# ahmetumutdurmus/zaremba

Hardware: NVIDIA H100
Metric: tokens/sec (and valid perplexity) Large-LSTM 1500h at 1/2/4/8 H100 vs ref CPU (higher is better)
Workload: dtype f16 operands, f32 accumulate/state

## Files before the change

zaremba_b200/csrc/engine_tc.cu:

```cuda
#include "engine.h"
#include <stdlib.h>
#include <string.h>

#include "tc_kernels.h"

struct GridBarrier {
    unsigned int* word = nullptr;
    unsigned int base = 0;
    template <typename Launch>
    int claim(int T, int nCTA, cudaStream_t s, Launch&& launch) {
        const unsigned int arrivals = (unsigned int)T * (unsigned int)nCTA;
        if (base > 0xF0000000u - arrivals) {
            ZRB_CUDA(cudaMemsetAsync(word, 0, sizeof(unsigned int), s));
            base = 0;
        }
        ZRB_TRY(launch(word, base));
        base += arrivals;
        return ZRB_OK;
    }
};

struct zrb_tc_state {
    int Xp[ZRB_MAX_LAYERS + 1] = {}, G4p[ZRB_MAX_LAYERS] = {}, Vp = 0;
    int Fp = 0;
// ... 213 lines not shown
    zrb_tc_state::WhhImage w;
    if (wd_mask(c, l).active) {
        w.kind = zrb_tc_state::kWhhMasked;
        w.seed = c->wd_seed; w.step = c->step; w.p = c->p_wd;
    }
    return w;
}
static bool whh_current(const zrb_ctx* c, int l) {
    const zrb_tc_state::WhhImage &have = c->tc->whh_img[l], want = whh_wanted(c, l);
    if (have.kind != want.kind) return false;
    return want.kind == zrb_tc_state::kWhhRaw || (have.seed == want.seed && have.step == want.step && have.p == want.p);
}

static int tc_pack_whh(zrb_ctx* c, const float* W, int l, bool row_image, cudaStream_t s) {
    const int H = c->width[l + 1];
    const MaskSrc m = wd_mask(c, l);
    const WeightImages w = c->tc->w_hh_images(l, whh_wanted(c, l), row_image);
    if (w.row) ZRB_TRY(convert_pad_f16(W, H, w.row, w.ld, 4 * H, H, 1.f, s, m));
    if (w.fwd) ZRB_TRY(pack_whh_fwd(W, w.fwd, H, *w.fplan, s, m));
    if (w.bwd) ZRB_TRY(pack_whh_bwd(W, w.bwd, H, *w.bplan, s, m));
    return ZRB_OK;
}

static size_t params_bytes(const zrb_ctx* c) { return c->experts ? sizeof(zrb_mos_params) : sizeof(zrb_params); }
static void note_packed(zrb_ctx* c, const zrb_params* p) {
    zrb_tc_state* t = c->tc;
    t->packed_version = c->weights_version;
    memcpy(&t->packed_params, p, params_bytes(c));
}

static int tc_pack_weights(zrb_ctx* c, const zrb_params* p, cudaStream_t s) {
    zrb_tc_state* t = c->tc;
    if (t->packed_version == c->weights_version && !memcmp(&t->packed_params, p, params_bytes(c))) return ZRB_OK;
    ProfScope ps(c, ZRB_PROF_PACK, s);
    const int L = c->cfg.layers, V = c->cfg.vocab;
    for (int l = 0; l < L; ++l) {
        const int In = c->width[l], H = c->width[l + 1];
        ZRB_TRY(convert_pad_f16(p->w_ih[l], In, t->w_ih_h[l], t->Xp[l], 4 * H, In, 1.f, s));
        ZRB_TRY(tc_pack_whh(c, p->w_hh[l], l, true, s));
    }
    const int F = c->experts ? c->width[0] : c->width[L];
    ZRB_TRY(convert_pad_f16(p->fc_w, F, t->fc_w_h, t->Fp, V, F, 1.f, s));
    if (c->experts) {
        const int K = c->experts, H = c->width[L];
        const zrb_mos_params* mp = mos_of(p);
        ZRB_TRY(convert_pad_f16(mp->latent_w, H, t->head_w_h, t->Xp[L], K * c->width[0], H, 1.f, s));
        ZRB_TRY(convert_pad_f16(mp->prior_w, H, t->head_w_h + (size_t)t->Ua * t->Xp[L], t->Xp[L], K, H, 1.f, s));
    }
    note_packed(c, p);
    return ZRB_OK;
}

struct WeightMatrix {
    int i, rows, cols, item;
    enum { kWih, kWhh, kFcW, kPrior, kLatent } kind;
};
struct WeightMatrices {
    WeightMatrix m[2 * ZRB_MAX_LAYERS + 3];
    int n = 0;
    const WeightMatrix* begin() const { return m; }
    const WeightMatrix* end() const { return m + n; }
    const WeightMatrix& fc_w() const { return m[n - 1]; }
};
static WeightMatrices tc_matrices(const zrb_ctx* c) {
    const int L = c->cfg.layers, V = c->cfg.vocab, K = c->experts;
    WeightMatrices ms;
    for (int l = 0; l < L; ++l) {
        const int In = c->width[l], H = c->width[l + 1];
        ms.m[ms.n++] = {1 + 4 * l, 4 * H, In, l, WeightMatrix::kWih};
        ms.m[ms.n++] = {2 + 4 * l, 4 * H, H, l, WeightMatrix::kWhh};
    }
    if (K) {
        ms.m[ms.n++] = {3 + 4 * L, K, c->width[L], L, WeightMatrix::kPrior};
        ms.m[ms.n++] = {4 + 4 * L, K * c->width[0], c->width[L], L, WeightMatrix::kLatent};
    }
    ms.m[ms.n++] = {1 + 4 * L, V, K ? c->width[0] : c->width[L], L, WeightMatrix::kFcW};
    return ms;
}
static WeightImages tc_images(zrb_ctx* c, const WeightMatrix& m, const zrb_tc_state::WhhImage& whh) {
    zrb_tc_state* t = c->tc;
    switch (m.kind) {
        case WeightMatrix::kWhh: return t->w_hh_images(m.item, whh);
        case WeightMatrix::kWih: return t->w_ih_images(m.item);
        case WeightMatrix::kFcW: return t->fc_w_images();
        case WeightMatrix::kPrior: return t->row_image(t->head_w_h + (size_t)t->Ua * t->Xp[m.item], t->Xp[m.item]);
        default: return t->row_image(t->head_w_h, t->Xp[m.item]);
    }
}
static TensorList tc_without_matrices(const zrb_ctx* c, const TensorList& tl) {
    TensorList rest = tl;
    for (const WeightMatrix& m : tc_matrices(c)) rest.n[m.i] = 0;
    return rest;
}
static void tc_images_current(zrb_ctx* c, const zrb_params* p) {
    zrb_tc_state* t = c->tc;
    t->wg_ok = false;
    c->weights_version++;
    note_packed(c, p);
}

static int tc_update_matrix(zrb_ctx* c, const WeightMatrix& m, const UpdateStep& st, int pdl_smem, cudaStream_t s) {
    zrb_tc_state::WhhImage whh;
    if (st.train() && c->p_wd > 0.f) whh.kind = zrb_tc_state::kWhhStale;
    const WeightImages img = tc_images(c, m, whh);
    float *p = st.tl.p[m.i], *g = st.tl.g[m.i];
    switch (st.kind) {
        case UpdateStep::kSgd:
            return update_pack(p, g, m.rows, m.cols, st.lr, c->scalars, img, c->keep_clipped, s, pdl_smem);
        case UpdateStep::kSgdAvg:
            return update_pack_avg(p, g, st.avg.a[m.i], st.avg.mu, st.avg.first, m.rows, m.cols, st.lr, c->scalars, img,
                                   c->keep_clipped, s, pdl_smem);
        case UpdateStep::kAdam:
            return update_pack_adam(p, g, st.adam.m[m.i], st.adam.v[m.i], st.adam.k, m.rows, m.cols, c->scalars, img,
                                    c->keep_clipped, s, pdl_smem);
        case UpdateStep::kDyn:
            return update_pack_dyn(p, g, st.tg[m.i], st.r[m.i], m.rows, m.cols, st.dyn, img, s);
        case UpdateStep::kSwap:
            return swap_pack(p, st.avg.a[m.i], m.rows, m.cols, img, s);
    }
    return ZRB_E_INVALID;
}

static int tc_issue_update(zrb_ctx* c, int item, int pdl_smem, cudaStream_t s) {
    zrb_tc_state* t = c->tc;
    if (!(t->upd_pending & (1u << item))) return ZRB_OK;
    t->upd_pending &= ~(1u << item);
    for (const WeightMatrix& m : tc_matrices(c))
        if (m.item == item) ZRB_TRY(tc_update_matrix(c, m, t->upd, pdl_smem, s));
    return ZRB_OK;
}

int tc_flush_updates(zrb_ctx* c, cudaStream_t s) {
    zrb_tc_state* t = c->tc;
    if (!t || !t->upd_pending) return ZRB_OK;
    ProfScope ps(c, ZRB_PROF_CLIP_SGD, s);
    for (int item = 1; item <= c->cfg.layers; ++item) ZRB_TRY(tc_issue_update(c, item, 0, s));
    return ZRB_OK;
}

static int tc_mos_head(zrb_ctx* c, const zrb_params* p, int rows, float* logp, cudaStream_t s) {
    zrb_tc_state* t = c->tc;
    const int L = c->cfg.layers, V = c->cfg.vocab, K = c->experts, E = c->width[0], H = c->width[L];
    const int N = c->T * c->B, Xl = t->Xp[L], Ep = pad64(E);
    ProfScope ps(c, ZRB_PROF_PROJ_FWD, s);
    Gemm head;
    head.A = {t->x_h[L] + (size_t)(N - rows) * Xl, Xl}; head.B = {t->head_w_h, Xl};
    head.C = t->ua; head.ldc = t->HW; head.M = rows; head.N = t->Ua + K; head.K = H;
    ZRB_TRY(gemm_f16_tc(head, s));
    ZRB_TRY(mos_latent_fwd(t->ua, t->HW, mos_of(p)->latent_b, t->lat_h, Ep, rows, K, E, N - rows, mos_mask(c), s));
    Gemm logits;
    logits.A = {t->lat_h, Ep}; logits.B = {t->fc_w_h, t->Fp};
    logits.C = t->logits; logits.ldc = V; logits.M = rows * K; logits.N = V; logits.K = E; logits.bias = p->fc_b;
    ZRB_TRY(gemm_f16_tc(logits, s));
    ZRB_TRY(mos_lse(t->logits, rows * K, V, t->lse, s));
    if (logp) ZRB_TRY(mos_logp(t->logits, t->lse, t->ua, t->HW, t->Ua, rows, K, V, logp, V, s));
    return ZRB_OK;
}

int tc_forward(zrb_ctx* c, const zrb_params* p, const int64_t* x, const zrb_states* in, const zrb_states* out,
               float* scores, cudaStream_t s, bool last_only) {
    zrb_tc_state* t = c->tc;
    const int L = c->cfg.layers, V = c->cfg.vocab, T = c->T, B = c->B, N = T * B;
    const bool ride = t->upd_pending && t->in_train_step && t->fplan[0].ok && pdl_beside_rec(c);
    if (t->upd_pending && !ride) ZRB_TRY(tc_flush_updates(c, s));
    ZRB_TRY(tc_pack_weights(c, p, s));
    {
        FwdPrep fp = {};
        for (int l = 0; l < L; ++l) {
            fp.in_h[l] = in->h[l]; fp.in_c[l] = in->c[l]; fp.h0s[l] = c->h0s[l]; fp.c0s[l] = c->c0s[l];
            fp.hprev_h[l] = t->hprev_h[l]; fp.h0_img[l] = t->fplan[l].ok ? t->h0_img[l] : nullptr;
            fp.rm[l] = rec_mask(c, l);
            fp.H[l] = c->width[l + 1]; fp.Hp[l] = t->Xp[l + 1]; fp.GB[l] = t->fplan[l].GBi; fp.Kc[l] = t->fplan[l].Kc;
        }
        fp.x = x; fp.x_saved = c->x_saved;
        fp.L = L; fp.B = B; fp.N = N;
        ZRB_TRY(fwd_prep(fp, s));
    }
    ZRB_TRY(zoneout_draw(c, s));
    {
        ProfScope ps(c, ZRB_PROF_EMBED_FWD, s);
        const bool through = ride && c->tied && (t->upd_pending & (1u << L));
        ZRB_TRY(embed_dropout_fwd(p->embed_w, x, nullptr, t->x_h[0], t->Xp[0], N, c->width[0], V, site_mask(c, 0), ed_mask(c), s,
                                  through ? t->upd.tl.g[tc_matrices(c).fc_w().i] : nullptr, t->upd.lr, c->scalars));
    }
    for (int l = 0; l < L; ++l) {
        const int In = c->width[l], H = c->width[l + 1], Xi = t->Xp[l], Hp = t->Xp[l + 1];
        const size_t bh = (size_t)B * H * sizeof(float);
        const RecPlan& fplan = t->fplan[l];
        float* G = c->gates[l];
        if (!whh_current(c, l)) {
            ProfScope ps(c, ZRB_PROF_PACK, s);
            ZRB_TRY(tc_pack_whh(c, p->w_hh[l], l, false, s));
        }
        {
            ProfScope ps(c, ZRB_PROF_GEMM_IN, s);
            Gemm xw;
            xw.A = {t->x_h[l], Xi}; xw.B = {t->w_ih_h[l], Xi};
            xw.C = G; xw.ldc = 4 * H; xw.M = N; xw.N = 4 * H; xw.K = In; xw.bias = p->b_ih[l]; xw.bias2 = p->b_hh[l];
            ZRB_TRY(gemm_f16_tc(xw, s));
        }
        MaskSrc m = site_mask(c, l + 1), rm = rec_mask(c, l);
        const ZoneoutSrc zo = zoneout_src(c, l);
        const bool reg_h = t->in_train_step && reg_on(c) && l == L - 1;
        ProfScope ps(c, ZRB_PROF_REC_FWD, s);
        if (fplan.ok) {
            ZRB_TRY(t->fwd_bar.claim(T, fplan.nCTA, s, [&](unsigned int* word, unsigned int base) {
                RecFwdArgs a = {};
                a.w_img = t->w_img_f[l]; a.h0_img = t->h0_img[l]; a.h_img = t->h_img; a.gates = G; a.c0 = c->c0s[l];
                a.cst = c->cst[l]; a.h_last = out->h[l]; a.c_last = out->c[l]; a.hprev_h = t->hprev_h[l];
                a.y_h = t->x_h[l + 1]; a.h_f32 = reg_h ? c->hraw[l] : nullptr; a.counter = word; a.base = base;
                a.T = T; a.B = B; a.H = H; a.Hp = Hp; a.m = m; a.rm = rm; a.trace = t->trace;
                a.zo = zo; a.h0 = c->h0s[l]; a.ctil = c->ctil[l];
                return lstm_rec_fwd(fplan, tc_watchdog(c), a, s);
            }));
            if (ride) ZRB_TRY(tc_issue_update(c, l + 1, fplan.beside_smem, s));
            continue;
        }
        for (int tt = 0; tt < T; ++tt) {
            const float* c_prev = tt ? c->cst[l] + (size_t)(tt - 1) * B * H : c->c0s[l];
            float* Gt = G + (size_t)tt * B * 4 * H;
            Gemm hw;
            hw.A = {t->hprev_h[l] + (size_t)tt * B * Hp, Hp}; hw.B = {t->w_hh_h[l], Hp};
            hw.C = Gt; hw.ldc = 4 * H; hw.M = B; hw.N = 4 * H; hw.K = H; hw.accumulate = true;
            ZRB_TRY(gemm_f16_tc(hw, s));
            const float* h_prev = tt ? c->hraw[l] + (size_t)(tt - 1) * B * H : c->h0s[l];
            ZRB_TRY(lstm_cell_fwd_tc(Gt, c_prev, c->cst[l] + (size_t)tt * B * H, c->hraw[l] + (size_t)tt * B * H,
                                     t->hprev_h[l] + (size_t)(tt + 1) * B * Hp, t->x_h[l + 1] + (size_t)tt * B * Hp, Hp, B,
                                     H, (int64_t)tt * B * H, (int64_t)N * H, m, rm, s, zo.on ? &zo : nullptr, h_prev,
                                     zo.on ? c->ctil[l] + (size_t)tt * B * H : nullptr));
        }
        ZRB_CUDA(cudaMemcpyAsync(out->h[l], c->hraw[l] + (size_t)(T - 1) * B * H, bh, cudaMemcpyDeviceToDevice, s));
        ZRB_CUDA(cudaMemcpyAsync(out->c[l], c->cst[l] + (size_t)(T - 1) * B * H, bh, cudaMemcpyDeviceToDevice, s));
    }
    if (scores && c->experts) return tc_mos_head(c, p, last_only ? B : N, t->head_loss_only ? nullptr : scores, s);
    if (scores) {
        ProfScope ps(c, ZRB_PROF_PROJ_FWD, s);
        const int rows = last_only ? B : N;
        const int Xl = t->Xp[L];
        Gemm proj;
        proj.A = {t->x_h[L] + (size_t)(N - rows) * Xl, Xl}; proj.B = {t->fc_w_h, Xl};
        proj.C = scores; proj.ldc = V; proj.M = rows; proj.N = V; proj.K = c->width[L]; proj.bias = p->fc_b;
        ZRB_TRY(gemm_f16_tc(proj, s));
    }
    return ZRB_OK;
}

const __half* tc_last_layer_image(const zrb_ctx* c) { return c->tc->x_h[c->cfg.layers]; }

static float* wgrad_slots(zrb_ctx* c, int n) {
    zrb_tc_state* t = c->tc;
    if (!t->wg_ok) return nullptr;
    if (t->wg_slots + n > kNormGemm) {
        t->wg_ok = false;
        return nullptr;
    }
    float* out = c->partials + norm_partials_base() + kNormExtra + t->wg_slots;
    t->wg_slots += n;
    return out;
}
static float* wgrad_sumsq(zrb_ctx* c, const Gemm& d) { return wgrad_slots(c, gemm_f16_tc_sumsq_slots(d).first); }

static int tc_mos_backward(zrb_ctx* c, const zrb_params* g, float* dY, cudaStream_t s) {
    zrb_tc_state* t = c->tc;
    const int L = c->cfg.layers, V = c->cfg.vocab, N = c->T * c->B, H = c->width[L], K = c->experts, E = c->width[0];
    const int NK = N * K, Xl = t->Xp[L], Vp = t->Vp, Ep = pad64(E);
// ... 365 lines not shown
    dw.dual.B = t->hprev_h[0]; dw.dual.C = dw_hh; dw.dual.N = H; dw.dual.ldb = Hp; dw.dual.ldc = H;
    ZRB_TRY(gemm_f16_tc(dw, s));
    c->layer_fwd_ok = false;
    return ZRB_OK;
}

int tc_rec_trace(zrb_ctx* c, long long* h_out, int max_entries) {
    if (!c->tc || !c->tc->trace) { set_error("set ZRB_REC_TRACE=1 before creating the context"); return ZRB_E_STATE; }
    int n = 2 * (8 + c->cfg.max_seq * 8);
    if (n > max_entries) n = max_entries;
    ZRB_CUDA(cudaDeviceSynchronize());
    ZRB_CUDA(cudaMemcpy(h_out, c->tc->trace, (size_t)n * sizeof(long long), cudaMemcpyDeviceToHost));
    return n;
}

int tc_apply_update(zrb_ctx* c, const zrb_params* p, const UpdateStep& st, float max_norm, float* norm_out,
                    cudaStream_t s) {
    zrb_tc_state* t = c->tc;
    const TensorList& tl = st.tl;
    const int E = c->width[0], V = c->cfg.vocab, L = c->cfg.layers;
    const bool adam = st.kind == UpdateStep::kAdam;
    ZRB_TRY(tc_flush_updates(c, s));
    ProfScope ps(c, st.kind == UpdateStep::kSwap ? ZRB_PROF_PACK : ZRB_PROF_CLIP_SGD, s);
    TensorList rest = tc_without_matrices(c, tl);
    bool lazy = false;
    if (st.train()) {
        const bool rows_only = !c->tied && c->emb_sparse && c->emb_prev_grad == tl.g[0] && c->emb_prev_n > 0;
        const bool gemm_norm = t->wg_ok && t->wg_key == tl.g[tc_matrices(c).fc_w().i];
        if (rows_only && !adam) rest.n[0] = 0;
        TensorList dense = gemm_norm ? rest : tl;
        if (rows_only) dense.n[0] = 0;
        if (c->tied && gemm_norm) {
            ZRB_TRY(grad_norm(dense, max_norm, c->partials, c->scalars, norm_out, s, true, t->wg_slots));
        } else if (rows_only) {
            ZRB_TRY(embed_first_table(c->emb_prev_ids, c->emb_first, c->emb_prev_n, V, s));
            ZRB_TRY(embed_rows_sumsq(tl.g[0], c->emb_prev_ids, c->emb_first, c->emb_prev_n, E, V,
                                     c->partials + norm_partials_base(), kNormExtra, s));
            ZRB_TRY(grad_norm(dense, max_norm, c->partials, c->scalars, norm_out, s, true, gemm_norm ? t->wg_slots : 0));
            if (!adam)
                ZRB_TRY(embed_rows_update(tl.p[0], tl.g[0], c->emb_prev_ids, c->emb_first, c->emb_prev_n, E, V, st.lr,
                                          c->scalars, c->keep_clipped, s));
            if (st.kind == UpdateStep::kSgdAvg) {
                TensorList e{};
                e.p[0] = tl.p[0]; e.n[0] = tl.n[0]; e.count = 1;
                ZRB_TRY(avg_apply(e, st.avg.a, st.avg.mu, st.avg.first, s));
            }
        } else {
            ZRB_TRY(grad_norm(tl, max_norm, c->partials, c->scalars, norm_out, s));
        }
        lazy = c->lazy_update && t->persistent() && pdl_beside_rec(c);
        if (lazy) t->upd = st;
    }
    for (const WeightMatrix& m : tc_matrices(c)) {
        if (lazy && m.item >= 1 && !(adam && c->tied && m.item == L)) t->upd_pending |= 1u << m.item;
        else ZRB_TRY(tc_update_matrix(c, m, st, 0, s));
    }
    ZRB_TRY(update_list(c, st, rest, s));
    tc_images_current(c, p);
    return ZRB_OK;
}

}
```

zaremba_b200/csrc/gemm_tc.cu:

```cuda
#include <stdlib.h>
#include <string.h>

#include "kernels.h"
#include "tc_common.cuh"
#include "tc_host.h"

namespace zrb {

using namespace tc;

constexpr int GBM = 128, GBK = 64;
constexpr int kASubBytes = GBM * GBK * 2;
constexpr int kEpiWarps = 8;
constexpr int kGemmThreads = 3 * 128;
template <int GBN> struct GemmCfg {
    static constexpr int kStages = GBN == 256 ? 4 : 6;
    static constexpr int kABytes = kASubBytes;
    static constexpr int kBBytes = GBN * GBK * 2;
    static constexpr int kSmem = kStages * (kABytes + kBBytes) + 1024  + 256 ;
};

struct GemmArgs {
    int M, N, K;
    float alpha;
// ... 391 lines not shown
    static EncodeTiledFn fn = nullptr;
    static bool tried = false;
    if (!tried) {
        tried = true;
        void* p = nullptr;
        cudaDriverEntryPointQueryResult q;
        if (cudaGetDriverEntryPoint("cuTensorMapEncodeTiled", &p, cudaEnableDefault, &q) == cudaSuccess &&
            q == cudaDriverEntryPointSuccess)
            fn = (EncodeTiledFn)p;
    }
    return fn;
}

int g_num_sms = 0;
bool g_attr_set[64][8] = {};

}

int tc_num_sms() {
    if (!g_num_sms) {
        int dev = 0;
        cudaGetDevice(&dev);
        cudaDeviceGetAttribute(&g_num_sms, cudaDevAttrMultiProcessorCount, dev);
        if (g_num_sms <= 0) g_num_sms = 132;
    }
    return g_num_sms;
}

int tc_make_tmap_f16(CUtensorMap* m, const void* ptr, uint64_t inner, uint64_t outer, uint64_t ld, uint32_t box_inner,
                     uint32_t box_outer, int swizzle128) {
    EncodeTiledFn enc = get_encode();
    if (!enc) {
        set_error("cuTensorMapEncodeTiled not available from the driver");
        return ZRB_E_CUDA;
    }
    ZRB_REQUIRE((ld * 2) % 16 == 0 && (((uintptr_t)ptr) & 15) == 0, "TMA operand needs 16-byte aligned base and pitch");
    cuuint64_t dims[2] = {inner, outer};
    cuuint64_t strides[1] = {ld * 2};
    cuuint32_t box[2] = {box_inner, box_outer};
    cuuint32_t estr[2] = {1, 1};
    CUresult r = enc(m, CU_TENSOR_MAP_DATA_TYPE_FLOAT16, 2, const_cast<void*>(ptr), dims, strides, box, estr,
                     CU_TENSOR_MAP_INTERLEAVE_NONE, swizzle128 ? CU_TENSOR_MAP_SWIZZLE_128B : CU_TENSOR_MAP_SWIZZLE_NONE,
                     CU_TENSOR_MAP_L2_PROMOTION_L2_256B, CU_TENSOR_MAP_FLOAT_OOB_FILL_NONE);
    if (r != CUDA_SUCCESS) {
        set_error("cuTensorMapEncodeTiled failed (%d) inner=%llu outer=%llu ld=%llu", (int)r,
                  (unsigned long long)inner, (unsigned long long)outer, (unsigned long long)ld);
        return ZRB_E_CUDA;
    }
    return ZRB_OK;
}

template <bool A_MN, bool B_MN, int GBN>
static int launch_gemm(const CUtensorMap& ta, const CUtensorMap& tb, const CUtensorMap& tb2, const GemmArgs& a,
                       cudaStream_t s) {
    auto kern = gemm_f16_tc_kernel<A_MN, B_MN, GBN>;
    const int idx = (A_MN ? 2 : 0) + (B_MN ? 1 : 0) + (GBN == 256 ? 4 : 0);
    int dev = 0;
    cudaGetDevice(&dev);
    dev &= 63;
    if (!g_attr_set[dev][idx]) {
        ZRB_CUDA(cudaFuncSetAttribute(kern, cudaFuncAttributeMaxDynamicSharedMemorySize, GemmCfg<GBN>::kSmem));
        g_attr_set[dev][idx] = true;
    }
    const int work = a.C2 ? a.tiles_m * (a.tiles_n + a.tiles_n2) : a.tiles_m * a.tiles_n * a.splits;
    int grid = work;
    if (grid > tc_num_sms()) grid = tc_num_sms();
    if (a.pdl_tail) {
        grid = work;
        cudaLaunchConfig_t cfg = {};
        cfg.gridDim = dim3(grid); cfg.blockDim = dim3(kGemmThreads);
        cfg.dynamicSmemBytes = GemmCfg<GBN>::kSmem; cfg.stream = s;
        cudaLaunchAttribute at[1];
        at[0].id = cudaLaunchAttributeProgrammaticStreamSerialization;
        at[0].val.programmaticStreamSerializationAllowed = 1;
        cfg.attrs = at; cfg.numAttrs = 1;
        ZRB_CUDA(cudaLaunchKernelEx(&cfg, kern, ta, tb, tb2, a));
        count_launch();
        return ZRB_OK;
    }
    kern<<<grid, kGemmThreads, GemmCfg<GBN>::kSmem, s>>>(ta, tb, tb2, a);
    ZRB_KERNEL_CHECK();
    return ZRB_OK;
}

static const void* pair_kernel(bool a_mn, bool b_mn) {
    if (!a_mn) return b_mn ? (const void*)gemm_f16_tc_pair_kernel<false, true> : (const void*)gemm_f16_tc_pair_kernel<false, false>;
    return b_mn ? (const void*)gemm_f16_tc_pair_kernel<true, true> : (const void*)gemm_f16_tc_pair_kernel<true, false>;
}

static void pair_launch_config(cudaLaunchConfig_t* cfg, cudaLaunchAttribute* cluster, int grid) {
    *cfg = {};
    cfg->gridDim = dim3(grid); cfg->blockDim = dim3(kGemmThreads); cfg->dynamicSmemBytes = PairCfg::kSmem;
    cluster->id = cudaLaunchAttributeClusterDimension;
    cluster->val.clusterDim.x = 2; cluster->val.clusterDim.y = 1; cluster->val.clusterDim.z = 1;
    cfg->attrs = cluster; cfg->numAttrs = 1;
}

static int g_pair_clusters[64][4] = {};

static bool pair_plan_fits(int pairs, bool a_mn, bool b_mn) {
    int dev = 0;
    cudaGetDevice(&dev);
    int& slot = g_pair_clusters[dev & 63][(a_mn ? 2 : 0) + (b_mn ? 1 : 0)];
    if (!slot) {
        const void* kern = pair_kernel(a_mn, b_mn);
        cudaLaunchConfig_t cfg;
        cudaLaunchAttribute cluster;
        pair_launch_config(&cfg, &cluster, tc_num_sms() & ~1);
        int n = 0;
        if (cudaFuncSetAttribute(kern, cudaFuncAttributeMaxDynamicSharedMemorySize, PairCfg::kSmem) != cudaSuccess ||
            cudaOccupancyMaxActiveClusters(&n, kern, &cfg) != cudaSuccess) {
            (void)cudaGetLastError();
            n = 0;
        }
        slot = 1 + n;
    }
    return pairs <= slot - 1;
}

static int launch_gemm_pair(const CUtensorMap& ta, const CUtensorMap& tb, const GemmArgs& a, int pairs, bool a_mn,
                            bool b_mn, cudaStream_t s) {
    cudaLaunchConfig_t cfg;
    cudaLaunchAttribute cluster;
    pair_launch_config(&cfg, &cluster, 2 * pairs);
    cfg.stream = s;
    void* args[] = {(void*)&ta, (void*)&tb, (void*)&a};
    ZRB_CUDA(cudaLaunchKernelExC(&cfg, pair_kernel(a_mn, b_mn), args));
    count_launch();
    return ZRB_OK;
}

template <int GBN>
static int dispatch_gemm(const CUtensorMap& ta, const CUtensorMap& tb, const CUtensorMap& tb2, const GemmArgs& a,
                         int a_mn, int b_mn, cudaStream_t s) {
    if (!a_mn && !b_mn) return launch_gemm<false, false, GBN>(ta, tb, tb2, a, s);
    if (!a_mn && b_mn) return launch_gemm<false, true, GBN>(ta, tb, tb2, a, s);
    if (a_mn && !b_mn) return launch_gemm<true, false, GBN>(ta, tb, tb2, a, s);
    return launch_gemm<true, true, GBN>(ta, tb, tb2, a, s);
}

struct TileChoice { int bn, tiles_m, tiles_n, splits; };
static TileChoice choose_tiles(int M, int N, int num_kb, bool can_split, bool retile = false) {
    const int nsm = tc_num_sms();
    TileChoice c;
    c.tiles_m = cdiv(M, GBM);
    const int t256 = c.tiles_m * cdiv(N, 256);
    if (can_split && t256 * 2 <= nsm && t256 * 2 >= (nsm * 4) / 10 && num_kb / 2 >= 8) {
        c.bn = 256; c.tiles_n = cdiv(N, 256); c.splits = 2;
        return c;
    }
    c.bn = (t256 >= (nsm * 9) / 10) ? 256 : 128;
    if (retile && c.bn == 256 && cdiv(t256, nsm) * 2 > cdiv(c.tiles_m * cdiv(N, 128), nsm) &&
             c.tiles_m * cdiv(N, 128) * 2 > nsm)
        c.bn = 128;
    c.tiles_n = cdiv(N, c.bn);
    c.splits = (can_split && c.tiles_m * c.tiles_n * 2 <= nsm && num_kb >= 8) ? 2 : 1;
    return c;
}

static TileChoice gemm_tiles(const Gemm& g, bool sumsq, bool direct) {
    if (g.dual.C) return choose_tiles(g.M, g.N > g.dual.N ? g.N : g.dual.N, cdiv(g.K, GBK), false);
    const bool plain = !sumsq && !g.accumulate;
    return choose_tiles(g.M, g.N, cdiv(g.K, GBK), plain && g.ldc == g.N, plain && !direct);
}

GemmSlots gemm_f16_tc_sumsq_slots(const Gemm& g) {
    const TileChoice c = gemm_tiles(g, true, false);
    GemmSlots n;
    n.first = c.tiles_m * cdiv(g.N, c.bn) * kEpiWarps;
    n.dual = g.dual.C ? c.tiles_m * cdiv(g.dual.N, c.bn) * kEpiWarps : 0;
    return n;
}

int gemm_f16_tc(const Gemm& g, cudaStream_t s) {
    const int M = g.M, N = g.N, K = g.K;
    const Gemm::Dual& d2 = g.dual;
    if (M <= 0 || N <= 0) return ZRB_OK;
    ZRB_REQUIRE(!d2.B == !d2.C, "dual launch needs both B2 and C2");
    ZRB_REQUIRE(!d2.C || (d2.N > 0 && !g.bias && !g.accumulate), "dual launch: N2 > 0, no bias, no accumulate");
    ZRB_REQUIRE(!g.bias2 || g.bias, "bias2 needs bias");
    ZRB_REQUIRE(!g.sumsq || !g.accumulate, "sumsq_out needs a plain store epilogue");
    ZRB_REQUIRE(K > 0, "gemm_f16_tc needs K > 0");
    const char* epi = getenv("ZRB_GEMM_EPI");
    const bool direct = epi && strcmp(epi, "direct") == 0;
    const TileChoice tc = gemm_tiles(g, g.sumsq != nullptr, direct);
    const int bn = tc.bn;
    const bool a_mn = g.A.mn_major, b_mn = g.B.mn_major;
    const int tiles_m64 = cdiv(M, PBM);
    const int pairs = 2 * pairs_per_split(tiles_m64, tc.tiles_n);
    const bool paired = !direct && tc.splits == 2 && bn == 256 && !g.a_tiled && !g.b_tiled && tiles_m64 > tc.tiles_m &&
                        pair_plan_fits(pairs, a_mn, b_mn);
    const int box_m = paired ? PBM : GBM, box_n = paired ? bn / 2 : bn;
    CUtensorMap ta, tb;
    if (!a_mn) ZRB_TRY(tc_make_tmap_f16(&ta, g.A.ptr, K, M, g.A.ld, GBK, box_m, 1));
    else       ZRB_TRY(tc_make_tmap_f16(&ta, g.A.ptr, M, K, g.A.ld, 64, GBK, 1));
    if (!b_mn) ZRB_TRY(tc_make_tmap_f16(&tb, g.B.ptr, K, N, g.B.ld, GBK, box_n, 1));
    else       ZRB_TRY(tc_make_tmap_f16(&tb, g.B.ptr, N, K, g.B.ld, 64, GBK, 1));
    CUtensorMap tb2 = tb;
    if (d2.B) {
        if (!b_mn) ZRB_TRY(tc_make_tmap_f16(&tb2, d2.B, K, d2.N, d2.ldb, GBK, bn, 1));
        else       ZRB_TRY(tc_make_tmap_f16(&tb2, d2.B, d2.N, K, d2.ldb, 64, GBK, 1));
    }
    GemmArgs a;
    a.M = M; a.N = N; a.K = K; a.alpha = g.alpha; a.bias = g.bias; a.C = g.C; a.ldc = g.ldc;
    a.accumulate = g.accumulate;
    a.tiles_m = tc.tiles_m; a.tiles_n = cdiv(N, bn);
    a.splits = tc.splits;
    a.sumsq_out = g.sumsq;
    a.bias2 = g.bias2;
    a.C2 = d2.C; a.sumsq_out2 = d2.sumsq;
    a.N2 = d2.N; a.ldc2 = d2.ldc; a.tiles_n2 = cdiv(d2.N, bn);
    a.a_tiled = a_mn ? nullptr : g.a_tiled; a.a_nt128 = g.a_nt128; a.b_tiled = b_mn ? nullptr : g.b_tiled;
    a.b_nt128 = g.b_nt128;
    a.pdl_tail = (g.pdl && a.splits == 1) ? 1 : 0;
    a.pdl_trigger = (rec_pdl_enabled() && !a.pdl_tail) ? 1 : 0;
    a.epi_direct = direct ? 1 : 0;
    if (a.splits > 1 && !g.accumulate) ZRB_CUDA(cudaMemsetAsync(g.C, 0, (size_t)M * N * sizeof(float), s));
    if (paired) {
        a.tiles_m = tiles_m64;
        return launch_gemm_pair(ta, tb, a, pairs, a_mn, b_mn, s);
    }
    return bn == 256 ? dispatch_gemm<256>(ta, tb, tb2, a, a_mn, b_mn, s) : dispatch_gemm<128>(ta, tb, tb2, a, a_mn, b_mn, s);
}

}

extern "C" int zrb_gemm_f16_tiled(const void* A, int64_t lda, const void* B, int64_t ldb, const void* A_tiled, int32_t a_nt128,
                                  const void* B_tiled, int32_t b_nt128, float* C, int64_t ldc, int32_t M, int32_t N, int32_t K,
                                  float alpha, void* stream) {
    ZRB_REQUIRE(A && B && C, "null argument");
    zrb::Gemm g;
    g.A = {(const __half*)A, lda}; g.B = {(const __half*)B, ldb};
    g.C = C; g.ldc = ldc; g.M = M; g.N = N; g.K = K; g.alpha = alpha;
    g.a_tiled = (const __half*)A_tiled; g.a_nt128 = a_nt128; g.b_tiled = (const __half*)B_tiled; g.b_nt128 = b_nt128;
    return zrb::gemm_f16_tc(g, (cudaStream_t)stream);
}

extern "C" int zrb_gemm_f16(const void* A, int64_t lda, int32_t a_mn_major, const void* B, int64_t ldb,
                            int32_t b_mn_major, float* C, int64_t ldc, int32_t M, int32_t N, int32_t K, float alpha,
                            const float* bias, int32_t accumulate, void* stream) {
    ZRB_REQUIRE(A && B && C, "null argument");
    zrb::Gemm g;
    g.A = {(const __half*)A, lda, a_mn_major != 0}; g.B = {(const __half*)B, ldb, b_mn_major != 0};
    g.C = C; g.ldc = ldc; g.M = M; g.N = N; g.K = K; g.alpha = alpha; g.bias = bias; g.accumulate = accumulate != 0;
    return zrb::gemm_f16_tc(g, (cudaStream_t)stream);
}
```

zaremba_b200/csrc/lstm_rec_fwd.cuh:

```cuda
#pragma once
#include "rec_common.cuh"

namespace zrb {


__device__ __forceinline__ uint32_t fwd_cluster_ctarank() {
    uint32_t r;
    asm volatile("mov.u32 %0, %%cluster_ctarank;" : "=r"(r));
    return r;
}
__device__ __forceinline__ uint32_t fwd_mapa(uint32_t local_addr, uint32_t rank) {
    uint32_t r;
    asm volatile("mapa.shared::cluster.u32 %0, %1, %2;" : "=r"(r) : "r"(local_addr), "r"(rank));
    return r;
}
__device__ __forceinline__ void fwd_cluster_sync() {
    asm volatile("barrier.cluster.arrive.release.aligned;\n\tbarrier.cluster.wait.acquire.aligned;" ::: "memory");
}

template <bool SPLIT, bool ZO>
__global__ void __launch_bounds__(kRecThreads, 1) lstm_rec_fwd_kernel(RecFwdArgs a) {
    extern __shared__ uint8_t smem_raw[];
    uint8_t* smem = smem_raw + ((128u - (smem_u32(smem_raw) & 127u)) & 127u);
    const int a_bytes = a.KcS * a.G * 128;
    const int b_bytes = a.KcS * a.GBi * 128;
    const int Bp = a.GBi * 8;
    const int ldd = Bp + 1;
    const int ldr = Bp + 4;
    uint8_t* sA = smem;
    uint8_t* sB = smem + a_bytes;
    float* sD = (float*)(sB + b_bytes);
    float* sR = sD;
    uint64_t* bars = (uint64_t*)((uint8_t*)sD + 2 * 64 * ldd * 4);
    uint64_t* bar_a = bars;
    uint64_t* bar_b = bars + 1;
    uint64_t* bar_mma = bars + 1 + kRecPieces;
    uint64_t* bar_recv = bar_mma + 1;

    const int warp = __shfl_sync(0xffffffffu, (int)(threadIdx.x >> 5), 0);
    const int lane = threadIdx.x & 31;
    const int cta = blockIdx.x;
    const uint32_t rank = SPLIT ? fwd_cluster_ctarank() : 0u;
    const int j0 = cta * a.U;
    const int nu = max(0, min(a.U, a.H - j0));
    const int ksteps = a.KcS / 2;
    const int piece_steps = (ksteps + kRecPieces - 1) / kRecPieces;
    const bool tr = a.trace != nullptr && cta == 0;
    long long* const trs = a.trace + 8;
    if (a.trace && threadIdx.x == 0) rec_launch_stamps(a.trace, tr, false);

    if (threadIdx.x == 0) {
        mbar_init(bar_a, 1);
        for (int i = 0; i < kRecPieces; ++i) mbar_init(&bar_b[i], 1);
        mbar_init(bar_mma, kRecMmaThreads);
        mbar_init(bar_recv, 1);
        fence_mbar_init();
    }
    __syncthreads();
    if (SPLIT) fwd_cluster_sync();

    if (warp == kRecLoadWarp && lane == 0) {
        const uint8_t* src = (const uint8_t*)a.w_img + (size_t)cta * a_bytes;
        mbar_expect_tx(bar_a, a_bytes);
        for (int off = 0; off < a_bytes; off += 32768) bulk_load_1d(sA + off, src + off, min(32768, a_bytes - off), bar_a);
        pdl_wait();
        bool dead = false;
        const int lbo_b = a.GBi * 128;
        const size_t img_bytes = (size_t)a.Kc * a.GBi * 128;
        for (int t = 0; t < a.T; ++t) {
            if (t > 0) grid_counter_wait(a.counter, a.base + (unsigned int)t * a.nCTA, a.w, dead, t);
            if (dead) break;
            if (tr) trs[t * 8 + 0] = clock64();
            fence_proxy_async_global();
            const uint8_t* img = (t == 0 ? (const uint8_t*)a.h0_img : (const uint8_t*)a.h_img + (size_t)t * img_bytes) +
                                 (size_t)rank * b_bytes;
            for (int pc = 0; pc < kRecPieces; ++pc) {
                const int k0 = pc * piece_steps, k1 = min(ksteps, k0 + piece_steps);
                if (k0 >= k1) { mbar_arrive(&bar_b[pc]); continue; }
                const int off = k0 * 2 * lbo_b, bytes = (k1 - k0) * 2 * lbo_b;
                mbar_expect_tx(&bar_b[pc], bytes);
                bulk_load_1d(sB + off, img + off, bytes, &bar_b[pc]);
            }
        }
    } else if (warp >= kRecMmaWarp && warp < kRecMmaWarp + kRecMmaWarps) {
        const uint32_t a_addr = smem_u32(sA), b_addr = smem_u32(sB);
        const uint32_t lbo_a = a.G * 128, lbo_b = a.GBi * 128;
        const int rows_pair = 8 * a.U;
        const int mt = SPLIT && rows_pair > 64 ? 2 : 1;
        const uint32_t sR_addr = smem_u32(sR), bar_recv_addr = smem_u32(bar_recv);
        const int tm = (int)threadIdx.x - kRecMmaWarp * 32;
        uint32_t row_dst[2][2], row_owner[2][2], row_bar[2][2];
        bool row_ok[2][2];
#pragma unroll
        for (int m = 0; m < 2; ++m)
#pragma unroll
            for (int h = 0; h < 2; ++h) {
                const int row = rec_acc_row(tm, m, h);
                if (!SPLIT) {
                    row_dst[m][h] = (uint32_t)(row * ldd * 4);
                    row_owner[m][h] = 0u; row_bar[m][h] = 0u; row_ok[m][h] = true;
                } else {
                    const int up = row >> 2, owner = up / a.U, lrow = (row & 3) * a.U + (up - owner * a.U);
                    row_ok[m][h] = row < rows_pair;
                    row_owner[m][h] = row_ok[m][h] ? (uint32_t)owner : 0u;
                    row_dst[m][h] = sR_addr + (uint32_t)(((int)rank * 4 * a.U + lrow) * ldr * 4);
                    row_bar[m][h] = fwd_mapa(bar_recv_addr, row_owner[m][h]);
                }
            }
        bool dead = false;
        bounded_mbar_wait(bar_a, 0, a.w, dead, kWaitWeights, 0);
        dead = rec_mma_any(dead);
        auto emit = [&](int m, int h, int col, float v0, float v1) {
            if (!SPLIT) {
                float* dst = (float*)((uint8_t*)sD + row_dst[m][h]) + col;
                dst[0] = v0;
// ... 135 lines not shown
```

zaremba_b200/csrc/tc_host.h:

```cpp
#pragma once
#include <cuda.h>
#include <cuda_fp16.h>

#include "common.cuh"

namespace zrb {
int tc_num_sms();
int tc_make_tmap_f16(CUtensorMap* m, const void* ptr, uint64_t inner, uint64_t outer, uint64_t ld, uint32_t box_inner,
                     uint32_t box_outer, int swizzle128);
struct GemmOperand {
    const __half* ptr = nullptr;
    int64_t ld = 0;
    bool mn_major = false;
};
struct Gemm {
    GemmOperand A, B;
    float* C = nullptr;
    int64_t ldc = 0;
    int M = 0, N = 0, K = 0;
    float alpha = 1.f;
    const float* bias = nullptr;
    const float* bias2 = nullptr;
    bool accumulate = false;
    float* sumsq = nullptr;
    bool pdl = false;
    struct Dual {
        const __half* B = nullptr;
        float* C = nullptr;
        int N = 0;
        int64_t ldb = 0, ldc = 0;
        float* sumsq = nullptr;
    } dual;
    const __half* a_tiled = nullptr;
    int a_nt128 = 0;
    const __half* b_tiled = nullptr;
    int b_nt128 = 0;
};
int gemm_f16_tc(const Gemm& g, cudaStream_t s);
struct GemmSlots {
    int first, dual;
};
GemmSlots gemm_f16_tc_sumsq_slots(const Gemm& g);
}
```

zaremba_b200/csrc/tc_kernels.h:

```cpp
#pragma once
#include "kernels.h"
#include "tc_host.h"

namespace zrb {

constexpr float kGradScale = 1024.f;

int convert_pad_f16(const float* src, int64_t ld_src, __half* dst, int64_t ld_dst, int rows, int cols, float scale,
                    cudaStream_t s, MaskSrc m = MaskSrc{});
int colsum_h_scratch_floats(int M);
int colsum_h(const __half* A, int64_t ld, float* out, float* out2, int N, int M, float inv_scale, float* scratch,
             cudaStream_t s);

int mos_latent_fwd(float* ua, int64_t ldu, const float* b, __half* lat_h, int64_t ld_l, int rows, int K, int E,
                   int64_t row0, MaskSrc m, cudaStream_t s);
int mos_latent_bwd(const float* dlat, const float* ua, int64_t ldu, __half* dua_h, int64_t ld_d, int N, int K, int E,
                   MaskSrc m, cudaStream_t s);
int mos_lse(const float* Z, int rows, int V, float* lse, cudaStream_t s);
int mos_nll_grad(const float* Z, const float* lse, const float* ua, int64_t ldu, int Ua, const int64_t* y, int N, int K,
                 int V, int B, float* row_loss, float* loss, __half* ds_h, int64_t ld_s, __half* dua_h, int64_t ld_d,
                 cudaStream_t s);
int mos_nll_eval(const float* Z, const float* lse, const float* ua, int64_t ldu, int Ua, const int64_t* y, int N, int K,
                 int V, int B, float* row_loss, float* loss, float* tgt_prob, cudaStream_t s);
int mos_logp(const float* Z, const float* lse, const float* ua, int64_t ldu, int Ua, int rows, int K, int V, float* out,
// ... 24 lines not shown
    int GB;
    int Kc;
    int nCTA;
    int smem;
    int KS;
    int KcS;
    int GBi;
    const void* kernel;
    int cluster;
    int max_clusters;
    int beside_smem;
};
size_t rec_smem_bytes(int Kc, int G, int GB);
int rec_split_groups(int GB);
int rec_max_clusters(const void* kernel, int cluster, int smem, int nCTA);
int rec_plan_finish(RecPlan* plan, const void* kernel, int cluster);
int rec_launch(const RecPlan& p, void** args, bool trace, cudaStream_t s, const char* name);
const void* rec_fwd_zoneout_kernel(bool split);
const void* rec_bwd_zoneout_kernel(int S);
struct RecWatchdog {
    unsigned int* flag = nullptr;
    unsigned int* host = nullptr;
};
struct RecWatch {
    unsigned int* flag;
    unsigned int* host;
    long long spin_cycles;
};
int rec_fwd_plan(int H, int B, RecPlan* plan);
int pack_whh_fwd(const float* W, __half* img, int H, const RecPlan& p, cudaStream_t s, MaskSrc m = MaskSrc{});
struct RecFwdArgs {
    const __half* w_img;
    const __half* h0_img;
    __half* h_img;
    float* gates;
    const float* c0;
    float* cst;
    float* h_last;
    float* c_last;
    __half* hprev_h;
    __half* y_h;
    float* h_f32;
    unsigned int* counter;
    unsigned int base;
    int T, B, H, Hp, U, G, GB, Kc, nCTA;
    int KcS, GBi;
    MaskSrc m;
    MaskSrc rm;
    RecWatch w;
    long long* trace;
    ZoneoutSrc zo;
    const float* h0;
    float* ctil;
};
int lstm_rec_fwd(const RecPlan& p, const RecWatchdog& wd, RecFwdArgs a, cudaStream_t s);
struct FwdPrep {
    const float* in_h[ZRB_MAX_LAYERS];
    const float* in_c[ZRB_MAX_LAYERS];
    float* h0s[ZRB_MAX_LAYERS];
    float* c0s[ZRB_MAX_LAYERS];
    __half* hprev_h[ZRB_MAX_LAYERS];
    __half* h0_img[ZRB_MAX_LAYERS];
    MaskSrc rm[ZRB_MAX_LAYERS];
    const int64_t* x;
    int64_t* x_saved;
    int H[ZRB_MAX_LAYERS], Hp[ZRB_MAX_LAYERS];
    int GB[ZRB_MAX_LAYERS], Kc[ZRB_MAX_LAYERS];
    int L, B, N;
};
int fwd_prep(const FwdPrep& a, cudaStream_t s);
struct WeightImages {
    __half* row = nullptr;
    int64_t ld = 0;
    __half* fwd = nullptr;
    const RecPlan* fplan = nullptr;
    __half* bwd = nullptr;
    const RecPlan* bplan = nullptr;
};
int update_pack(float* p, float* g, int rows, int cols, float lr, const float* scalars, const WeightImages& img,
                bool write_g, cudaStream_t s,
                int pdl_smem = 0);
int update_pack_dyn(float* p, float* g, const float* tg, const float* r, int rows, int cols, const DynArgs& a,
                    const WeightImages& img, cudaStream_t s);
int update_pack_avg(float* p, float* g, float* a, float mu, bool first, int rows, int cols, float lr,
                    const float* scalars, const WeightImages& img, bool write_g, cudaStream_t s, int pdl_smem = 0);
int update_pack_adam(float* p, float* g, float* m, float* v, const AdamScalars& k, int rows, int cols,
                     const float* scalars, const WeightImages& img, bool write_g, cudaStream_t s, int pdl_smem = 0);
int swap_pack(float* p, float* a, int rows, int cols, const WeightImages& img, cudaStream_t s);
int rec_bwd_plan(int H, int B, RecPlan* plan);
int pack_whh_bwd(const float* W, __half* img, int H, const RecPlan& p, cudaStream_t s, MaskSrc m = MaskSrc{});
struct RecBwdArgs {
    const __half* w_img;
    __half* g_img;
    const float* dy;
    const float* r;
    const float* gates;
    const float* cst;
    const float* c0;
    __half* dG_h;
    float* db1;
    float* db2;
    float* db_scratch;
    unsigned int* counter;
    unsigned int base;
    int T, B, H, G4p, U, G, GB, Kc, nCTA;
    int KcS, GBi;
// ... 11 lines not shown
```

Measured before the change: 440,300.

## Defer layer-0 W_hh update to run beside the first input-projection GEMM

The lazy SGD update for layer 0's recurrent weight matrix gets its own pending item. When weight decay is off, it is issued right after the layer-0 input-projection GEMM, sized to fit in the shared memory that GEMM leaves free. That GEMM is launched with the fewest CTAs that keep the same number of waves, leaving SM room for the update to overlap. The recurrent forward kernel then waits on PDL before bulk-loading its weight image, so it reads the freshly updated W_hh. This hides the update's cost inside the GEMM, but the recurrence can no longer prefetch weights before the dependency wait.

Result: faster. 447,800 (median of 6 runs) (+1.7%).

```diff
diff --git a/zaremba_b200/csrc/engine_tc.cu b/zaremba_b200/csrc/engine_tc.cu
--- a/zaremba_b200/csrc/engine_tc.cu
+++ b/zaremba_b200/csrc/engine_tc.cu
@@ -289,7 +289,7 @@
 }
 
 struct WeightMatrix {
-    int i, rows, cols, item;
+    int i, rows, cols, layer, item;
     enum { kWih, kWhh, kFcW, kPrior, kLatent } kind;
 };
 struct WeightMatrices {
@@ -299,29 +299,30 @@
     const WeightMatrix* end() const { return m + n; }
     const WeightMatrix& fc_w() const { return m[n - 1]; }
 };
+static int whh0_item(const zrb_ctx* c) { return c->cfg.layers + 1; }
 static WeightMatrices tc_matrices(const zrb_ctx* c) {
     const int L = c->cfg.layers, V = c->cfg.vocab, K = c->experts;
     WeightMatrices ms;
     for (int l = 0; l < L; ++l) {
         const int In = c->width[l], H = c->width[l + 1];
-        ms.m[ms.n++] = {1 + 4 * l, 4 * H, In, l, WeightMatrix::kWih};
-        ms.m[ms.n++] = {2 + 4 * l, 4 * H, H, l, WeightMatrix::kWhh};
+        ms.m[ms.n++] = {1 + 4 * l, 4 * H, In, l, l, WeightMatrix::kWih};
+        ms.m[ms.n++] = {2 + 4 * l, 4 * H, H, l, l ? l : whh0_item(c), WeightMatrix::kWhh};
     }
     if (K) {
-        ms.m[ms.n++] = {3 + 4 * L, K, c->width[L], L, WeightMatrix::kPrior};
-        ms.m[ms.n++] = {4 + 4 * L, K * c->width[0], c->width[L], L, WeightMatrix::kLatent};
-    }
-    ms.m[ms.n++] = {1 + 4 * L, V, K ? c->width[0] : c->width[L], L, WeightMatrix::kFcW};
+        ms.m[ms.n++] = {3 + 4 * L, K, c->width[L], L, L, WeightMatrix::kPrior};
+        ms.m[ms.n++] = {4 + 4 * L, K * c->width[0], c->width[L], L, L, WeightMatrix::kLatent};
+    }
+    ms.m[ms.n++] = {1 + 4 * L, V, K ? c->width[0] : c->width[L], L, L, WeightMatrix::kFcW};
     return ms;
 }
 static WeightImages tc_images(zrb_ctx* c, const WeightMatrix& m, const zrb_tc_state::WhhImage& whh) {
     zrb_tc_state* t = c->tc;
     switch (m.kind) {
-        case WeightMatrix::kWhh: return t->w_hh_images(m.item, whh);
-        case WeightMatrix::kWih: return t->w_ih_images(m.item);
+        case WeightMatrix::kWhh: return t->w_hh_images(m.layer, whh);
+        case WeightMatrix::kWih: return t->w_ih_images(m.layer);
         case WeightMatrix::kFcW: return t->fc_w_images();
-        case WeightMatrix::kPrior: return t->row_image(t->head_w_h + (size_t)t->Ua * t->Xp[m.item], t->Xp[m.item]);
-        default: return t->row_image(t->head_w_h, t->Xp[m.item]);
+        case WeightMatrix::kPrior: return t->row_image(t->head_w_h + (size_t)t->Ua * t->Xp[m.layer], t->Xp[m.layer]);
+        default: return t->row_image(t->head_w_h, t->Xp[m.layer]);
     }
 }
 static TensorList tc_without_matrices(const zrb_ctx* c, const TensorList& tl) {
@@ -371,7 +372,7 @@
     zrb_tc_state* t = c->tc;
     if (!t || !t->upd_pending) return ZRB_OK;
     ProfScope ps(c, ZRB_PROF_CLIP_SGD, s);
-    for (int item = 1; item <= c->cfg.layers; ++item) ZRB_TRY(tc_issue_update(c, item, 0, s));
+    for (int item = 0; item <= whh0_item(c); ++item) ZRB_TRY(tc_issue_update(c, item, 0, s));
     return ZRB_OK;
 }
 
@@ -394,12 +395,15 @@
     return ZRB_OK;
 }
 
+static bool whh0_beside_gemm(const zrb_ctx* c) { return c->p_wd == 0.f; }
+
 int tc_forward(zrb_ctx* c, const zrb_params* p, const int64_t* x, const zrb_states* in, const zrb_states* out,
                float* scores, cudaStream_t s, bool last_only) {
     zrb_tc_state* t = c->tc;
     const int L = c->cfg.layers, V = c->cfg.vocab, T = c->T, B = c->B, N = T * B;
     const bool ride = t->upd_pending && t->in_train_step && t->fplan[0].ok && pdl_beside_rec(c);
     if (t->upd_pending && !ride) ZRB_TRY(tc_flush_updates(c, s));
+    if (!whh0_beside_gemm(c)) ZRB_TRY(tc_issue_update(c, whh0_item(c), 0, s));
     ZRB_TRY(tc_pack_weights(c, p, s));
     {
         FwdPrep fp = {};
@@ -425,6 +429,7 @@
         const size_t bh = (size_t)B * H * sizeof(float);
         const RecPlan& fplan = t->fplan[l];
         float* G = c->gates[l];
+        const bool whh0_beside = l == 0 && (t->upd_pending & (1u << whh0_item(c)));
         if (!whh_current(c, l)) {
             ProfScope ps(c, ZRB_PROF_PACK, s);
             ZRB_TRY(tc_pack_whh(c, p->w_hh[l], l, false, s));
@@ -434,8 +439,10 @@
             Gemm xw;
             xw.A = {t->x_h[l], Xi}; xw.B = {t->w_ih_h[l], Xi};
             xw.C = G; xw.ldc = 4 * H; xw.M = N; xw.N = 4 * H; xw.K = In; xw.bias = p->b_ih[l]; xw.bias2 = p->b_hh[l];
+            xw.fewest_ctas = whh0_beside;
             ZRB_TRY(gemm_f16_tc(xw, s));
         }
+        if (whh0_beside) ZRB_TRY(tc_issue_update(c, whh0_item(c), gemm_f16_tc_beside_smem(), s));
         MaskSrc m = site_mask(c, l + 1), rm = rec_mask(c, l);
         const ZoneoutSrc zo = zoneout_src(c, l);
         const bool reg_h = t->in_train_step && reg_on(c) && l == L - 1;
@@ -448,6 +455,7 @@
                 a.y_h = t->x_h[l + 1]; a.h_f32 = reg_h ? c->hraw[l] : nullptr; a.counter = word; a.base = base;
                 a.T = T; a.B = B; a.H = H; a.Hp = Hp; a.m = m; a.rm = rm; a.trace = t->trace;
                 a.zo = zo; a.h0 = c->h0s[l]; a.ctil = c->ctil[l];
+                a.w_after_wait = whh0_beside ? 1 : 0;
                 return lstm_rec_fwd(fplan, tc_watchdog(c), a, s);
             }));
             if (ride) ZRB_TRY(tc_issue_update(c, l + 1, fplan.beside_smem, s));
@@ -919,7 +927,9 @@
         if (lazy) t->upd = st;
     }
     for (const WeightMatrix& m : tc_matrices(c)) {
-        if (lazy && m.item >= 1 && !(adam && c->tied && m.item == L)) t->upd_pending |= 1u << m.item;
+        const bool defer = m.item >= 1 && !(adam && c->tied && m.item == L) &&
+                           (m.item != whh0_item(c) || whh0_beside_gemm(c));
+        if (lazy && defer) t->upd_pending |= 1u << m.item;
         else ZRB_TRY(tc_update_matrix(c, m, st, 0, s));
     }
     ZRB_TRY(update_list(c, st, rest, s));
diff --git a/zaremba_b200/csrc/gemm_tc.cu b/zaremba_b200/csrc/gemm_tc.cu
--- a/zaremba_b200/csrc/gemm_tc.cu
+++ b/zaremba_b200/csrc/gemm_tc.cu
@@ -467,7 +467,7 @@
 
 template <bool A_MN, bool B_MN, int GBN>
 static int launch_gemm(const CUtensorMap& ta, const CUtensorMap& tb, const CUtensorMap& tb2, const GemmArgs& a,
-                       cudaStream_t s) {
+                       bool fewest_ctas, cudaStream_t s) {
     auto kern = gemm_f16_tc_kernel<A_MN, B_MN, GBN>;
     const int idx = (A_MN ? 2 : 0) + (B_MN ? 1 : 0) + (GBN == 256 ? 4 : 0);
     int dev = 0;
@@ -480,6 +480,7 @@
     const int work = a.C2 ? a.tiles_m * (a.tiles_n + a.tiles_n2) : a.tiles_m * a.tiles_n * a.splits;
     int grid = work;
     if (grid > tc_num_sms()) grid = tc_num_sms();
+    if (fewest_ctas) grid = cdiv(work, cdiv(work, grid));
     if (a.pdl_tail) {
         grid = work;
         cudaLaunchConfig_t cfg = {};
@@ -547,11 +548,11 @@
 
 template <int GBN>
 static int dispatch_gemm(const CUtensorMap& ta, const CUtensorMap& tb, const CUtensorMap& tb2, const GemmArgs& a,
-                         int a_mn, int b_mn, cudaStream_t s) {
-    if (!a_mn && !b_mn) return launch_gemm<false, false, GBN>(ta, tb, tb2, a, s);
-    if (!a_mn && b_mn) return launch_gemm<false, true, GBN>(ta, tb, tb2, a, s);
-    if (a_mn && !b_mn) return launch_gemm<true, false, GBN>(ta, tb, tb2, a, s);
-    return launch_gemm<true, true, GBN>(ta, tb, tb2, a, s);
+                         int a_mn, int b_mn, bool fewest_ctas, cudaStream_t s) {
+    if (!a_mn && !b_mn) return launch_gemm<false, false, GBN>(ta, tb, tb2, a, fewest_ctas, s);
+    if (!a_mn && b_mn) return launch_gemm<false, true, GBN>(ta, tb, tb2, a, fewest_ctas, s);
+    if (a_mn && !b_mn) return launch_gemm<true, false, GBN>(ta, tb, tb2, a, fewest_ctas, s);
+    return launch_gemm<true, true, GBN>(ta, tb, tb2, a, fewest_ctas, s);
 }
 
 struct TileChoice { int bn, tiles_m, tiles_n, splits; };
@@ -635,7 +636,17 @@
         a.tiles_m = tiles_m64;
         return launch_gemm_pair(ta, tb, a, pairs, a_mn, b_mn, s);
     }
-    return bn == 256 ? dispatch_gemm<256>(ta, tb, tb2, a, a_mn, b_mn, s) : dispatch_gemm<128>(ta, tb, tb2, a, a_mn, b_mn, s);
+    return bn == 256 ? dispatch_gemm<256>(ta, tb, tb2, a, a_mn, b_mn, g.fewest_ctas, s)
+                     : dispatch_gemm<128>(ta, tb, tb2, a, a_mn, b_mn, g.fewest_ctas, s);
+}
+
+int gemm_f16_tc_beside_smem() {
+    int dev = 0, per_sm = 0, reserved = 0;
+    cudaGetDevice(&dev);
+    cudaDeviceGetAttribute(&per_sm, cudaDevAttrMaxSharedMemoryPerMultiprocessor, dev);
+    cudaDeviceGetAttribute(&reserved, cudaDevAttrReservedSharedMemoryPerBlock, dev);
+    const int smem = GemmCfg<128>::kSmem > GemmCfg<256>::kSmem ? GemmCfg<128>::kSmem : GemmCfg<256>::kSmem;
+    return per_sm - 2 * reserved - smem + 1;
 }
 
 }
diff --git a/zaremba_b200/csrc/lstm_rec_fwd.cuh b/zaremba_b200/csrc/lstm_rec_fwd.cuh
--- a/zaremba_b200/csrc/lstm_rec_fwd.cuh
+++ b/zaremba_b200/csrc/lstm_rec_fwd.cuh
@@ -61,6 +61,10 @@
 
     if (warp == kRecLoadWarp && lane == 0) {
         const uint8_t* src = (const uint8_t*)a.w_img + (size_t)cta * a_bytes;
+        if (a.w_after_wait) {
+            pdl_wait();
+            fence_proxy_async_global();
+        }
         mbar_expect_tx(bar_a, a_bytes);
         for (int off = 0; off < a_bytes; off += 32768) bulk_load_1d(sA + off, src + off, min(32768, a_bytes - off), bar_a);
         pdl_wait();
diff --git a/zaremba_b200/csrc/tc_host.h b/zaremba_b200/csrc/tc_host.h
--- a/zaremba_b200/csrc/tc_host.h
+++ b/zaremba_b200/csrc/tc_host.h
@@ -24,6 +24,7 @@
     bool accumulate = false;
     float* sumsq = nullptr;
     bool pdl = false;
+    bool fewest_ctas = false;
     struct Dual {
         const __half* B = nullptr;
         float* C = nullptr;
@@ -41,4 +42,5 @@
     int first, dual;
 };
 GemmSlots gemm_f16_tc_sumsq_slots(const Gemm& g);
+int gemm_f16_tc_beside_smem();
 }
diff --git a/zaremba_b200/csrc/tc_kernels.h b/zaremba_b200/csrc/tc_kernels.h
--- a/zaremba_b200/csrc/tc_kernels.h
+++ b/zaremba_b200/csrc/tc_kernels.h
@@ -100,6 +100,7 @@
     ZoneoutSrc zo;
     const float* h0;
     float* ctil;
+    int w_after_wait;
 };
 int lstm_rec_fwd(const RecPlan& p, const RecWatchdog& wd, RecFwdArgs a, cudaStream_t s);
 struct FwdPrep {
```
